# HKU-BAL/Clair3-RNA

Hardware: NVIDIA B200
Metric: candidate sites/sec (tensor+inference) (higher is better)
Workload: dtype int32 pileup + fp16/fp32-accumulate network

## Files before the change

### clair3_rna_b200/csrc/c3r_abi.cu

```cuda
#include <cstdio>
#include <cstdlib>
#include <cstring>
#include <string>
#include <vector>
#include <chrono>
#include <map>
#include <cuda_runtime.h>

#include "../../include/c3r_b200.h"
#include "pileup.cuh"
#include "nn_fp32.cuh"
#include "nn_tc.cuh"
#include "call.cuh"

using namespace c3r;

namespace {

struct Buf {
    void* p = nullptr;
    size_t cap = 0;
};
struct Pin {
    void* p = nullptr;
    size_t cap = 0;
};

constexpr int N_SLOTS = 4;
constexpr int N_EV = 9;

struct Slot {
    bool in_use = false;
    bool has_result = false;
    cudaStream_t st = nullptr;
    cudaStream_t st_a = nullptr;
    cudaEvent_t ev[N_EV] = {};
    cudaEvent_t ev_alt = nullptr;
    cudaEvent_t ev_call[2] = {};
    bool calls = false;
    Buf pos, flag, mapq, hp, cigar_off, cigar, seq_off, seq, ref;
    Buf admit, read_end, op_x, op_y, op_info, blockmax;
    Buf covA, covE, rowR, cov_up, ptile, ctile, csuper, word_base;
    Buf row_pos, counts, row_depth, row_flag, head_cnt, tail_cnt, skipdiff, max_skip, row_ins, row_del;
    Buf binc, bin_cur, events, raw, cov, cov_tile, refnib;
    Buf pbed, cbed, known, covP;
    Buf cand_row, cand_pos, cand_depth, tensor, alt_off, alt_n, alt, cur_ref, deleted, probs;
    Buf d_calls;
    Buf xop;
    bool fused_window = false;
    Buf scalars;
    Buf scan_scratch;
    ScanState scan = {};
    uint32_t scan_epoch = 0;
    size_t zero_bytes = 0;
    bool pending_b = false;
    cudaEvent_t ev_cnt = nullptr;
    uint64_t order = 0;
    int64_t n_seq_bytes = 0, n_known_sites = 0;
    bool exact_bounds = false;
    int deferred_rc = 0;
    std::string deferred_err;
    Pin h_scalars, h_pos, h_depth, h_probs, h_alt_off, h_alt_n, h_alt, h_tensor, h_row_pos, h_counts, h_row_depth, h_calls;
    Dev d;
    int64_t n_rows = 0, n_cand = 0, alt_total = 0;
    int launches = 0;
    c3r_result res;
};

}

struct c3r_ctx {
    int device = 0;
    c3r_params prm;
    std::string err;
    Slot slots[N_SLOTS];
    int sm_count = 148;
    bool have_weights = false;
// ... 57 lines not shown
    CK(cudaMallocHost(&b.p, want));
    b.cap = want;
    return 0;
}
void release(Buf& b) { if (b.p) cudaFree(b.p); b.p = nullptr; b.cap = 0; }
void release(Pin& b) { if (b.p) cudaFreeHost(b.p); b.p = nullptr; b.cap = 0; }

template <class T> T* P(Buf& b) { return (T*)b.p; }

__global__ void __launch_bounds__(128) k_call(const Dev d, const float* __restrict__ probs, int64_t n, c3r_call* __restrict__ out) {
    for (int64_t i = blockIdx.x * (int64_t)blockDim.x + threadIdx.x; i < n; i += (int64_t)gridDim.x * blockDim.x) {
        c3rcall::CallIn c;
        c.e = reinterpret_cast<const c3r_alt_entry*>(d.alt) + d.alt_off[i];
        c.n = d.alt_n[i];
        c.probs = probs + 24 * i;
        c.ref = d.ref;
        c.ref_len = d.ref_len;
        c.p0 = (int64_t)d.cand_pos[i] - (d.ref_start0 + 1);
        c.seq = d.seq;
        c3r_call r;
        c3rcall::decide_call(c, r);
        out[i] = r;
    }
}
static_assert(sizeof(AltEntry) == sizeof(c3r_alt_entry), "AltEntry mirrors c3r_alt_entry");

int run_stage_a(c3r_ctx* ctx, Slot& s) {
    Dev& d = s.d;
    cudaStream_t st = s.st_a;
    int& L = s.launches;
    CK(cudaMemsetAsync(s.covA.p, 0, s.zero_bytes, st));
    CK(cudaMemsetAsync(s.scalars.p, 0, 64, st));
    CK(cudaEventRecord(s.ev[1], st));
    if (d.n_reads > 0) {
        static const int force_g = getenv("C3R_CIGAR_G") ? atoi(getenv("C3R_CIGAR_G")) : 0;
        const int64_t avg = d.n_ops / d.n_reads;
        const int G = force_g ? force_g : avg >= 16 ? 32 : 8;
        if (G == 32) k_cigar<32><<<(unsigned)((d.n_reads * 32 + 255) / 256), 256, 0, st>>>(d);
        else if (G == 16) k_cigar<16><<<(unsigned)((d.n_reads * 16 + 255) / 256), 256, 0, st>>>(d);
        else k_cigar<8><<<(unsigned)((d.n_reads * 8 + 255) / 256), 256, 0, st>>>(d);
        ++L;
    }
    if (d.n_known > 0) { k_mark_known<<<(unsigned)((d.n_known + 255) / 256), 256, 0, st>>>(d); ++L; }
    const unsigned ptiles = (unsigned)((d.NW + PT_WORDS - 1) / PT_WORDS);
    k_row_bits<<<ptiles, 256, 0, st>>>(d); ++L;
    if (d.n_pbed >= 0) { k_bed_mask<<<(unsigned)((d.NW + 4 + 255) / 256), 256, 0, st>>>(d, (uint32_t*)s.covP.p); ++L; }
    if (d.head_tail) {
        k_last_col<<<(unsigned)((d.NW + 255) / 256), 256, 0, st>>>(d);
        k_last_gap<<<(unsigned)((d.NW + 255) / 256), 256, 0, st>>>(d);
        L += 2;
    }
    k_row_rank<<<ptiles, 256, 0, st>>>(d); ++L;
    CK(cudaEventRecord(s.ev[2], st));
    if (d.n_ops > 0) {
        const int64_t chunks = (d.n_ops + CMP_THREADS - 1) / CMP_THREADS;
        const int64_t cap = (int64_t)ctx->sm_count * 6;
        k_cmp<<<(unsigned)(chunks < cap ? chunks : cap), CMP_THREADS, 0, st>>>(d);
        ++L;
    }
    if (d.padding) { OpSkip op; op.d = d; L += device_scan(op, d.L_ub, s.scan, s.scan_epoch, (Int2*)nullptr, st); }
    { OpEvents op; op.d = d; L += device_scan(op, d.L_ub + 1, s.scan, s.scan_epoch, (int32_t*)nullptr, st); }
    if (d.C == 18) k_scatter_aggr<4><<<(unsigned)(ctx->sm_count * 8 + 1), 1024, 0, st>>>(d);
    else k_scatter_aggr<6><<<(unsigned)(ctx->sm_count * 8 + 1), 1024, 0, st>>>(d);
    ++L;
    CK(cudaEventRecord(s.ev[3], st));
    int64_t nb = (d.L_ub + COV_TILE - 1) / COV_TILE;
    {
        const int64_t res = (int64_t)ctx->sm_count * (d.C == 30 ? 4 : 5);
        const unsigned grid = (unsigned)(nb < res ? nb : res);
        if (d.C == 18) k_rows<18><<<grid, ROWS_WARPS * 32, 0, st>>>(d);
        else k_rows<30><<<grid, ROWS_WARPS * 32, 0, st>>>(d);
        ++L;
    }
    CK(cudaEventRecord(s.ev[4], st));
    k_cand_emit<<<(unsigned)(nb < ctx->sm_count * 16 ? nb : ctx->sm_count * 16), 256, 0, st>>>(d); ++L;
    CK(cudaEventRecord(s.ev[5], st));
    CK(cudaGetLastError());
    return 0;
}

int parse_scalars(c3r_ctx* ctx, Slot& s) {
    const int64_t* hs = (const int64_t*)s.h_scalars.p;
    s.n_rows = hs[0];
    s.n_cand = hs[1];
    const int32_t err = ((const int32_t*)s.h_scalars.p)[6];
    if (err == 7)
        return fail(ctx, C3R_ERR_CAPACITY, "a position is covered by more than 8000 reads: samtools mpileup (the reference's "
                                           "column source) caps the depth there and drops reads; this chunk is refused "
                                           "rather than called on different counts");
    if (err) {
// ... 180 lines not shown
        CK(cudaStreamCreateWithPriority(&s.st_a, cudaStreamNonBlocking, prio_lo));
        for (int k = 0; k < N_EV; ++k) CK(cudaEventCreate(&s.ev[k]));
        CK(cudaEventCreateWithFlags(&s.ev_alt, cudaEventDisableTiming));
        for (int k = 0; k < 2; ++k) CK(cudaEventCreate(&s.ev_call[k]));
        CK(cudaEventCreateWithFlags(&s.ev_cnt, cudaEventDisableTiming | (getenv("C3R_BLOCKING_COUNTS") ? cudaEventBlockingSync : 0)));
        if (ensure(ctx, s.scalars, 256)) return C3R_ERR_CUDA;
        if (ensure_pin(ctx, s.h_scalars, 256)) return C3R_ERR_CUDA;
    }
    CK(cudaStreamCreateWithFlags(&ctx->fwd_stream, cudaStreamNonBlocking));
    if (ensure(ctx, ctx->thr, 2 * THR_N * sizeof(uint16_t))) return C3R_ERR_CUDA;
    k_thr_table<<<(THR_N + 255) / 256, 256>>>((uint16_t*)ctx->thr.p, (uint16_t*)ctx->thr.p + THR_N, params->snp_min_af, params->indel_min_af);
    CK(cudaGetLastError());
    CK(cudaDeviceSynchronize());
    return C3R_OK;
}

void c3r_destroy(c3r_ctx* ctx) {
    if (!ctx) return;
    if (getenv("C3R_TIMING") && ctx->tc.pipe)
        fprintf(stderr, "[c3r] %ld network passes, %ld with LSTM1 in pieces beside the previous pass\n", ctx->tc.pipe->n_pass, ctx->tc.pipe->n_overlap);
    if (getenv("C3R_TIMING") && ctx->n_submit)
        fprintf(stderr, "[c3r] %lld submits, host ms each: buffers %.3f, h2d calls %.3f, stage A launches %.3f, earlier "
                        "tickets advanced at submit %.3f, deferred part (wait for the counts + stage B + d2h calls) %.3f, - %.3f\n", (long long)ctx->n_submit,
                1e3 * ctx->t_phase[0] / ctx->n_submit, 1e3 * ctx->t_phase[1] / ctx->n_submit, 1e3 * ctx->t_phase[2] / ctx->n_submit,
                1e3 * ctx->t_phase[3] / ctx->n_submit, 1e3 * ctx->t_phase[4] / ctx->n_submit, 1e3 * ctx->t_phase[5] / ctx->n_submit);
    cudaSetDevice(ctx->device);
    cudaDeviceSynchronize();
    if (ctx->nn_done) cudaEventDestroy(ctx->nn_done);
    for (int i = 0; i < N_SLOTS; ++i) {
        Slot& s = ctx->slots[i];
        Buf* bs[] = {&s.pos, &s.flag, &s.mapq, &s.hp, &s.cigar_off, &s.cigar, &s.seq_off, &s.seq, &s.ref, &s.admit,
                     &s.read_end, &s.op_x, &s.op_y, &s.op_info, &s.blockmax, &s.covA, &s.covE, &s.rowR, &s.cov_up, &s.ptile, &s.ctile, &s.csuper,
                     &s.word_base, &s.row_pos, &s.counts, &s.row_depth, &s.row_flag, &s.head_cnt, &s.tail_cnt,
                     &s.skipdiff, &s.max_skip, &s.row_ins, &s.row_del, &s.binc, &s.bin_cur, &s.events, &s.raw, &s.cov, &s.cov_tile, &s.refnib,
                     &s.cand_row, &s.cand_pos, &s.cand_depth, &s.tensor, &s.alt_off, &s.alt_n, &s.alt, &s.cur_ref,
                     &s.deleted, &s.probs, &s.scalars, &s.scan_scratch, &s.pbed, &s.cbed, &s.known, &s.covP, &s.xop, &s.d_calls};
        for (Buf* b : bs) release(*b);
        Pin* ps[] = {&s.h_scalars, &s.h_pos, &s.h_depth, &s.h_probs, &s.h_alt_off, &s.h_alt_n, &s.h_alt, &s.h_tensor,
                     &s.h_row_pos, &s.h_counts, &s.h_row_depth, &s.h_calls};
        for (Pin* b : ps) release(*b);
        for (int k = 0; k < N_EV; ++k) if (s.ev[k]) cudaEventDestroy(s.ev[k]);
        if (s.ev_alt) cudaEventDestroy(s.ev_alt);
        for (int k = 0; k < 2; ++k) if (s.ev_call[k]) cudaEventDestroy(s.ev_call[k]);
        if (s.ev_cnt) cudaEventDestroy(s.ev_cnt);
        if (s.st) cudaStreamDestroy(s.st);
        if (s.st_a) cudaStreamDestroy(s.st_a);
    }
    release(ctx->wbuf);
    release(ctx->nn_scratch);
    release(ctx->fwd_in);
    release(ctx->ref_res);
    release(ctx->refnib_res);
    release(ctx->thr);
    release(ctx->fwd_out);
    tc_release(ctx->tc);
    if (ctx->fwd_stream) cudaStreamDestroy(ctx->fwd_stream);
    delete ctx;
}

int c3r_host_alloc(void** out, int64_t n_bytes) {
    if (!out || n_bytes <= 0) return C3R_ERR_ARG;
    *out = nullptr;
    return cudaHostAlloc(out, (size_t)n_bytes, cudaHostAllocPortable) == cudaSuccess ? C3R_OK : C3R_ERR_CUDA;
}
void c3r_host_free(void* p) { if (p) cudaFreeHost(p); }

const char* c3r_last_error(c3r_ctx* ctx) { return ctx ? ctx->err.c_str() : "null context"; }
// ... 63 lines not shown
    ctx->filter = nullptr;
    return rc;
}

static int size_rows(c3r_ctx* ctx, Slot& s, const uint32_t* cigar_host) {
    Dev& d = s.d;
    int64_t md_len = 0, n_skip = 0, ev_ub = 0;
    if (cigar_host) {
        for (int64_t k = 0; k < d.n_ops; ++k) {
            const uint32_t c = cigar_host[k], op = c & 15u;
            const int64_t len = c >> 4;
            if (op == 0 || op == 2 || op == 7 || op == 8) md_len += len;
            if (op == 3) ++n_skip;
        }
        ev_ub = d.n_ops + 2 * s.n_seq_bytes;
    } else {
        md_len = 4 * s.n_seq_bytes;
        n_skip = d.n_ops;
        ev_ub = d.n_ops + s.n_seq_bytes / 2;
    }
    int64_t L_ub = md_len + 32 * (n_skip + d.n_reads) + 64;
    L_ub += 33 * s.n_known_sites;
    if (L_ub > d.W) L_ub = d.W;
    if (L_ub < 64) L_ub = 64;
    d.L_ub = L_ub;
    d.events_ub = ev_ub + 8;
    d.cand_cap = L_ub;
#define EN(b, bytes) if (ensure(ctx, s.b, (size_t)(bytes))) return C3R_ERR_CUDA
    EN(row_pos, (L_ub + 2) * 4); EN(counts, ((L_ub + 32) * d.C) * 4); EN(row_depth, (L_ub + 2) * 4); EN(row_flag, L_ub + 2);
    EN(head_cnt, (L_ub + 2) * 4); EN(tail_cnt, (L_ub + 2) * 4); EN(skipdiff, (L_ub + 2) * 8); EN(max_skip, (L_ub + 2) * 4);
    EN(row_ins, (L_ub + 2) * 4); EN(row_del, (L_ub + 2) * 4);
    EN(binc, (L_ub + 4) * 4); EN(bin_cur, (L_ub + 4) * 4);
    EN(events, d.events_ub * sizeof(RowEvent)); EN(raw, d.events_ub * sizeof(RowEvent));
    EN(cov, (L_ub + 4) * NCOV_MAX * 4); EN(cov_tile, (L_ub / COV_TILE + 4) * NCOV_MAX * 4);
    EN(ctile, (L_ub / COV_TILE + 4) * 4); EN(csuper, (L_ub / (64 * COV_TILE) + 4) * 4);
    EN(cand_row, (L_ub + 2) * 4); EN(cand_pos, (L_ub + 2) * 4); EN(cand_depth, (L_ub + 2) * 4);
    EN(cur_ref, (L_ub + 2) * 8); EN(deleted, L_ub + 2);
    {
        int64_t mx = d.n_ops > d.NW ? d.n_ops : d.NW;
        if (L_ub + 4 > mx) mx = L_ub + 4;
        const size_t tiles = (size_t)(mx / SCAN_TILE + 2);
        const size_t need = 256 + tiles * 4 + 2 * tiles * sizeof(ScanElem) + 64;
        if (s.scan_scratch.cap < need) {
            EN(scan_scratch, need);
            CK(cudaMemsetAsync(s.scan_scratch.p, 0, s.scan_scratch.cap, s.st_a));
        }
        uint8_t* sp = (uint8_t*)s.scan_scratch.p;
        const size_t cap_tiles = (s.scan_scratch.cap - 256 - 64) / (4 + 2 * sizeof(ScanElem));
        s.scan.ctrl = (unsigned int*)sp;
        s.scan.status = (uint32_t*)(sp + 256);
        s.scan.aggr = sp + 256 + ((cap_tiles * 4 + 15) / 16) * 16;
        s.scan.incl = (uint8_t*)s.scan.aggr + cap_tiles * sizeof(ScanElem);
        s.scan.err = P<int32_t>(s.scalars) + 6;
    }
#undef EN
    d.row_pos = P<int32_t>(s.row_pos); d.counts = P<int32_t>(s.counts); d.row_depth = P<int32_t>(s.row_depth);
    d.row_flag = P<uint8_t>(s.row_flag); d.head_cnt = P<int32_t>(s.head_cnt); d.tail_cnt = P<int32_t>(s.tail_cnt);
    d.skipdiff = P<Int2>(s.skipdiff); d.max_skip = P<int32_t>(s.max_skip);
    d.row_inscnt = P<int32_t>(s.row_ins); d.row_delcnt = P<int32_t>(s.row_del);
    d.binc = P<int32_t>(s.binc); d.bin_cur = P<int32_t>(s.bin_cur);
    d.events = P<RowEvent>(s.events); d.raw = P<RowEvent>(s.raw); d.cov = P<int32_t>(s.cov); d.cov_tile = P<int32_t>(s.cov_tile);
    d.ctile = P<int32_t>(s.ctile); d.csuper = P<int32_t>(s.csuper);
    d.cand_row = P<int32_t>(s.cand_row); d.cand_pos = P<int32_t>(s.cand_pos); d.cand_depth = P<int32_t>(s.cand_depth);
    d.cur_ref = P<Int2>(s.cur_ref); d.deleted = P<uint8_t>(s.deleted);
    return 0;
}

static int submit_once(c3r_ctx* ctx, const c3r_reads* rd, const uint8_t* ref, int64_t ref_start1, int64_t ref_len,
                       int64_t region_start1, int64_t region_end1, c3r_ticket* ticket) {
    if (!ref) {
        if (!ctx->ref_res_len) return fail(ctx, C3R_ERR_STATE, "ref == NULL but c3r_set_reference was never called");
        ref_start1 = ctx->ref_res_start0 + 1;
        ref_len = ctx->ref_res_len;
    }
    if (!ctx->have_weights) return fail(ctx, C3R_ERR_STATE, "c3r_set_weights must be called before c3r_submit_chunk");
    if (region_end1 < region_start1 || region_start1 < 1) return fail(ctx, C3R_ERR_ARG, "bad region");
    if (region_end1 > 0x7fff0000LL) return fail(ctx, C3R_ERR_CAPACITY, "positions must fit int32");
    if (rd->n_seq_bytes * 2 >= 0xffffffffLL) return fail(ctx, C3R_ERR_CAPACITY, "more than 4G bases in one chunk");
    if (rd->n_reads >= (1LL << 28)) return fail(ctx, C3R_ERR_CAPACITY, "more than 2^28 reads in one chunk");
    CK(cudaSetDevice(ctx->device));
    auto now = [] { return std::chrono::duration<double>(std::chrono::steady_clock::now().time_since_epoch()).count(); };
    double tp = now();
    auto lap = [&](int k) { const double t = now(); ctx->t_phase[k] += t - tp; tp = t; };
    ++ctx->n_submit;
    int si = -1;
    for (int i = 0; i < N_SLOTS; ++i) if (!ctx->slots[i].in_use) { si = i; break; }
    if (si < 0) return fail(ctx, C3R_ERR_STATE, "all tickets in flight; c3r_release one first");
    Slot& s = ctx->slots[si];
    s.launches = 0;
    s.has_result = false;
    s.calls = ctx->calls;
    Dev& d = s.d;
    memset(&d, 0, sizeof d);
    const c3r_params& pr = ctx->prm;
// ... 423 lines not shown
```

### clair3_rna_b200/csrc/pileup.cuh

```cuda
#pragma once
#include <cstdint>
#include <cuda_runtime.h>
#include <cuda_fp16.h>
#include "scan.cuh"

namespace c3r {

constexpr int MPILEUP_MAX_DEPTH = 8000;
constexpr int WIN = 33;
constexpr int FLANK = 16;
constexpr int TILE_ROWS = 32;
constexpr int COV_UP = 5;
constexpr int PT_WORDS = 1024;
constexpr uint32_t OP_SKIP = 0xffffffffu;
constexpr int COV_TILE = 256;

struct RowEvent {
    uint32_t info;
    int32_t len;
    uint32_t yb;
    int32_t row;
};

struct AltEntry {
// ... 15 lines not shown
struct Dev {
    int64_t n_reads, n_ops;
    const int32_t* pos; const uint16_t* flag; const uint8_t* mapq; const uint8_t* hp;
    const int32_t* cigar_off; const uint32_t* cigar; const int64_t* seq_off; const uint8_t* seq;
    const uint8_t* ref; int64_t ref_start0; int64_t ref_len;
    int32_t R0, R1; int64_t W; int64_t NW;
    int32_t C; int32_t min_cov; int32_t min_mq; uint32_t excl; double snp_af, indel_af;
    int32_t padding; int32_t max_depth; double skip_prop;
    int32_t dbg;

    const uint16_t* thr_snp; const uint16_t* thr_indel;
    const int32_t* pbed; int32_t n_pbed;
    const int32_t* cbed; int32_t n_cbed;
    const int32_t* known; int32_t n_known;
    const uint32_t* covP; int32_t head_tail;
    int32_t* tail;
    uint8_t* admit; int32_t* read_end;
    int32_t* op_x; uint32_t* op_y;
    uint32_t* op_info;
    uint32_t* covA; uint32_t* covE; uint32_t* rowR; int32_t* word_base;
    uint32_t* upA[COV_UP]; uint32_t* upE[COV_UP];
    int32_t* ptile;
    int32_t* kctr;
    int64_t L_ub;
    int64_t* n_rows;
    int32_t* row_pos; int32_t* counts; int32_t* row_depth; uint8_t* row_flag;
    int32_t* head_cnt; int32_t* tail_cnt; Int2* skipdiff; int32_t* max_skip;
    int32_t* row_inscnt; int32_t* row_delcnt;
    int32_t* binc; int32_t* bin_cur; RowEvent* events;
    RowEvent* raw; int64_t* n_raw;
    int64_t events_ub;
    int32_t* cov;
    int32_t* cov_tile;
    const uint32_t* refnib; int64_t n_ref_words;
    int32_t* blockmax;
    int32_t* ctile;
    int32_t* csuper;
    int64_t* n_cand; int32_t* cand_row; int64_t cand_cap;
    int32_t* cand_pos; int32_t* cand_depth;
    int32_t* tensor;
    int64_t* alt_off; int32_t* alt_n; AltEntry* alt; int64_t alt_cap;
    Int2* cur_ref; uint8_t* deleted;
    int32_t* err;
};

__device__ __forceinline__ bool op_consumes_ref(uint32_t op) { return op == 0 || op == 2 || op == 3 || op == 7 || op == 8; }
__device__ __forceinline__ bool op_consumes_qry(uint32_t op) { return op == 0 || op == 1 || op == 4 || op == 7 || op == 8; }
__device__ __forceinline__ bool op_is_match(uint32_t op) { return op == 0 || op == 7 || op == 8; }

__device__ __forceinline__ int32_t row_lower_bound(const Dev& d, int32_t p) {
    if (p <= d.R0) return 0;
    int64_t o = (int64_t)p - d.R0;
    if (o >= d.W) o = d.W;
    const int64_t w = o >> 5;
    const uint32_t m = (1u << (o & 31)) - 1u;
    return d.word_base[w] + __popc(d.rowR[w] & m);
}
__device__ __forceinline__ bool bit_at(const uint32_t* bm, int64_t o) { return (bm[o >> 5] >> (o & 31)) & 1u; }

__device__ __forceinline__ uint32_t nib_at(const uint8_t* seq, uint32_t q) {
    const uint32_t b = seq[q >> 1];
    return (q & 1u) ? (b & 15u) : (b >> 4);
}
__device__ __forceinline__ int ref_index(const Dev& d, int32_t p, bool* is_acgt) {
    const int64_t o = (int64_t)p - d.ref_start0;
    uint8_t c = (o >= 0 && o < d.ref_len) ? d.ref[o] : (uint8_t)'N';
// ... 253 lines not shown
    if (own) {
        int32_t idx = b;
#pragma unroll
        for (int j = 0; j < 4; ++j) {
            const int32_t p0 = d.R0 + (int32_t)((w4 + j) << 5);
            if (r[j] == 0xffffffffu) {
                for (int q = 0; q < 32; ++q) if (idx + q < d.L_ub) d.row_pos[idx + q] = p0 + q;
                idx += 32;
            } else {
                for (uint32_t m = r[j]; m; m &= m - 1) { if (idx < d.L_ub) d.row_pos[idx] = p0 + __ffs(m) - 1; ++idx; }
            }
        }
    }
    int64_t z0 = tile_base, z1 = tile_end;
    if (blockIdx.x == gridDim.x - 1) z1 += 2;
    if (z1 > d.L_ub + 2) z1 = d.L_ub + 2;
    for (int64_t i = z0 + t; i < z1; i += 256) {
        d.binc[i] = 0;
        d.bin_cur[i] = 0;
        for (int c = 0; c < NC; ++c) d.cov[i * NC + c] = 0;
        if (d.padding) {
            d.head_cnt[i] = 0; d.tail_cnt[i] = 0;
            Int2 z; z.a = 0; z.b = 0;
            d.skipdiff[i] = z;
            d.deleted[i] = 0;
        }
    }
    if (blockIdx.x == 0)
        for (int64_t i = t; i < d.L_ub / (64 * COV_TILE) + 2; i += 256) d.csuper[i] = 0;
    for (int64_t i = z0 / COV_TILE + t; i <= (z1 > z0 ? (z1 - 1) / COV_TILE : z0 / COV_TILE); i += 256) d.ctile[i] = 0;
    if (z1 > z0) {
        const int64_t ct0 = z0 / COV_TILE, ct1 = (z1 - 1) / COV_TILE + 1;
        for (int64_t i = ct0 * NC + t; i < (ct1 + 1) * NC; i += 256) d.cov_tile[i] = 0;
    }
}

__device__ __forceinline__ uint32_t nibmask(int n) {
    uint32_t m;
    asm("shl.b32 %0, 1, %1;" : "=r"(m) : "r"((uint32_t)(n < 0 ? 0 : 4 * n)));
    return m - 1u;
}

__global__ void k_refnib(const uint8_t* __restrict__ ref, int64_t ref_len, uint32_t* __restrict__ out, int64_t n_words) {
    const int64_t w = (int64_t)blockIdx.x * blockDim.x + threadIdx.x;
    if (w >= n_words) return;
    uint32_t v = 0;
#pragma unroll
    for (int j = 0; j < 8; ++j) {
        const int64_t o = w * 8 + j;
        uint8_t c = o < ref_len ? ref[o] : (uint8_t)'N';
        if (c >= 'a') c -= 32;
        const uint32_t nib = c == 'A' ? 1u : c == 'C' ? 2u : c == 'G' ? 4u : c == 'T' ? 8u : 0u;
        v |= nib << (4 * j);
    }
    out[w] = v;
}

constexpr int NCOV_MAX = 6;
constexpr int CMP_THREADS = 256;
constexpr int CMP_STAGE = 1536;

struct __align__(16) CmpOp {
    int32_t w0, w1;
    int32_t kw;
    uint32_t sh;
    int32_t rbase;
// ... 32 lines not shown
    const int32_t wi = w + c.kw;
    uint32_t f0, f1;
    if ((uint32_t)wi < (uint32_t)(d.n_ref_words - 1)) { f0 = d.refnib[wi]; f1 = d.refnib[wi + 1]; }
    else {
        f0 = (wi >= 0 && wi < d.n_ref_words) ? d.refnib[wi] : 0u;
        f1 = (wi + 1 >= 0 && wi + 1 < d.n_ref_words) ? d.refnib[wi + 1] : 0u;
    }
    uint32_t x = rw ^ __funnelshift_r(f0, f1, c.sh);
    x &= (w == c.w0 ? c.m0 : 0xffffffffu) & (w == c.w1 ? c.m1 : 0xffffffffu);
    if (x) cmp_emit(d, st, c, w, rw, x);
}

__device__ __forceinline__ void cmp_flush(const Dev& d, EventStage& st) {
    __syncthreads();
    const int n = st.n < CMP_STAGE ? st.n : CMP_STAGE;
    if (threadIdx.x == 0 && n > 0) st.base = (int)atomicAdd((unsigned long long*)d.n_raw, (unsigned long long)n);
    __syncthreads();
    if (n > 0) {
        const long long base = st.base;
        if (base + n > d.events_ub) { if (threadIdx.x == 0) atomicExch(d.err, 3); }
        else {
            for (int i = threadIdx.x; i < n; i += CMP_THREADS) {
                const RowEvent e = st.buf[i];
                d.raw[base + i] = e;
                atomicAdd(&d.binc[e.row], 1);
            }
        }
    }
    __syncthreads();
    if (threadIdx.x == 0) st.n = 0;
    __syncthreads();
}

__global__ void __launch_bounds__(CMP_THREADS) k_cmp(Dev d) {
    __shared__ EventStage st;
    __shared__ CmpOp wops[CMP_THREADS / 32][32];
    __shared__ int32_t wpre[CMP_THREADS / 32][32];
    const int lane = threadIdx.x & 31;
    const int NC = d.C == 30 ? 6 : 4;
    if (*d.err == 1) return;
    __shared__ int chunk_s;
    if (threadIdx.x == 0) st.n = 0;
    for (;;) {
    if (threadIdx.x == 0) chunk_s = atomicAdd(&d.kctr[3], 1);
    __syncthreads();
    const int64_t k0 = (int64_t)chunk_s * CMP_THREADS;
    if (k0 >= d.n_ops) break;
    const int64_t k = k0 + threadIdx.x;
    CmpOp cmp;
    cmp.w0 = 0; cmp.w1 = -1; cmp.kw = 0; cmp.sh = 0; cmp.rbase = 0; cmp.info = 0; cmp.m0 = 0; cmp.m1 = 0;
    do {
        if (k >= d.n_ops) break;
        const uint32_t oi = d.op_info[k];
        if (oi == OP_SKIP) break;
        const int32_t r = (int32_t)(oi >> 4);
        const uint32_t c = d.cigar[k];
        const uint32_t op = c & 15u;
        const int32_t len = (int32_t)(c >> 4);
        if (!op_consumes_ref(op) || len == 0) break;
        const int32_t x = d.op_x[k];
        const uint32_t rev = oi & 1u;
        const uint32_t hp = (oi >> 2) & 3u;
        const int32_t a = x < d.R0 ? d.R0 : x;
        const int32_t b = x + len > d.R1 ? d.R1 : x + len;

        if (op == 3) {
            if (d.padding && b > a) {
                const int32_t ra = row_lower_bound(d, a), rb = row_lower_bound(d, b);
                if (rb > ra) {
                    int32_t* f = rev ? &d.skipdiff[0].b : &d.skipdiff[0].a;
                    atomicAdd(&f[2 * (int64_t)ra], 1);
                    atomicAdd(&f[2 * (int64_t)rb], -1);
                }
            }
            break;
        }
        if (b > a) {
            const int32_t ra = row_lower_bound(d, a), rb = ra + (b - a);
            const int ch = (op == 2 ? 2 : 0) + (int)rev;
            atomicAdd(d.cov + (int64_t)ra * NC + ch, 1);
            atomicAdd(d.cov + (int64_t)rb * NC + ch, -1);
            const bool hpc = NC == 6 && op != 2 && hp;
            if (hpc) { atomicAdd(d.cov + (int64_t)ra * NC + 3 + hp, 1); atomicAdd(d.cov + (int64_t)rb * NC + 3 + hp, -1); }
            if (ra / COV_TILE != rb / COV_TILE) {
                atomicAdd(d.cov_tile + (int64_t)(ra / COV_TILE) * NC + ch, 1);
                atomicAdd(d.cov_tile + (int64_t)(rb / COV_TILE) * NC + ch, -1);
                if (hpc) {
                    atomicAdd(d.cov_tile + (int64_t)(ra / COV_TILE) * NC + 3 + hp, 1);
                    atomicAdd(d.cov_tile + (int64_t)(rb / COV_TILE) * NC + 3 + hp, -1);
                }
            }
            if (op != 2) {
                const int64_t qa = (int64_t)d.op_y[k] + (a - x);
                const int64_t qb = qa + (b - a);
                cmp.w0 = (int32_t)(qa >> 3); cmp.w1 = (int32_t)((qb - 1) >> 3);
                cmp.m0 = ~nibmask((int)(qa & 7)); cmp.m1 = nibmask((int)(qb - 8 * (int64_t)cmp.w1));
                const int64_t K = ((int64_t)a - d.ref_start0) - qa;
                cmp.kw = (int32_t)(K >> 3);
                cmp.sh = ((uint32_t)K & 7u) * 4u;
                cmp.rbase = (int32_t)((int64_t)ra - qa);
                cmp.info = oi & ~2u;
            }
        }
        if (d.padding) {
            if (x == d.pos[r] && x >= d.R0 && x < d.R1) {
                bool first = true;
                for (int32_t j = d.cigar_off[r]; j < k; ++j)
                    if (op_consumes_ref(d.cigar[j] & 15u) && (d.cigar[j] >> 4)) first = false;
                if (first) atomicAdd(&d.head_cnt[row_lower_bound(d, x)], 1);
            }
            const int32_t end = d.read_end[r];
            if (x + len == end && end - 1 >= d.R0 && end - 1 < d.R1)
                atomicAdd(&d.tail_cnt[row_lower_bound(d, end - 1)], 1);
        }
        const int32_t last = x + len - 1;
        if (last < d.R0 || last >= d.R1) break;
        if (oi & 2u) break;
        int64_t j = k + 1;
        bool more = true;
        int32_t ins_len = 0, del_len = 0;
        const uint32_t op2 = d.cigar[j] & 15u;
        if (op2 != 1 && !(op2 == 2 && op != 2)) break;
        if (op2 == 1) {
            while (more) {
                const uint32_t cj = d.cigar[j], o = cj & 15u;
                if (o == 1) ins_len += (int32_t)(cj >> 4);
                else if (o != 6) break;
                more = !(d.op_info[j] & 2u);
                ++j;
            }
        }
        if (more && (d.cigar[j] & 15u) == 2 && op != 2) {
            while (more) {
                const uint32_t cj = d.cigar[j];
                if ((cj & 15u) != 2) break;
                del_len += (int32_t)(cj >> 4);
                more = !(d.op_info[j] & 2u);
                ++j;
            }
        }
        if (!ins_len && !del_len) break;
        const int32_t row = row_lower_bound(d, last);
        for (int which = 0; which < 2; ++which) {
            const int32_t l = which ? del_len : ins_len;
            if (!l) continue;
            emit_event(d, st, row, ((uint32_t)r << 4) | (hp << 2) | ((uint32_t)which << 1) | rev, l,
                       d.op_y[k] + (op_is_match(op) ? (uint32_t)len : 0u));
        }
    } while (0);

    {
        const int warp = threadIdx.x >> 5;
        const int32_t cnt = cmp.w1 - cmp.w0 + 1;
        int32_t incl = cnt;
#pragma unroll
        for (int o = 1; o < 32; o <<= 1) { const int32_t y = __shfl_up_sync(0xffffffffu, incl, o); if (lane >= o) incl += y; }
        const int32_t total = __shfl_sync(0xffffffffu, incl, 31);
        wops[warp][lane] = cmp;
        wpre[warp][lane] = incl - cnt;
        __syncwarp();
        for (int32_t g = lane; g < total; g += 32) {
            int i = 0;
#pragma unroll
            for (int stp = 16; stp > 0; stp >>= 1) if (wpre[warp][i + stp] <= g) i += stp;
            const CmpOp c = wops[warp][i];
            cmp_one(d, st, c, c.w0 + (g - wpre[warp][i]));
        }
    }
    __syncthreads();
    const bool fl = st.n >= CMP_STAGE / 2;
    __syncthreads();
    if (fl) cmp_flush(d, st);
    }
    cmp_flush(d, st);
}

struct OpEvents {
    typedef int32_t T;
    struct Ctx {};
    Dev d;
    __device__ void ctx_init(Ctx&) const {}
    __device__ T identity() const { return 0; }
    __device__ T combine(const T& x, const T& y) const { return x + y; }
    __device__ int64_t size() const { return *d.n_rows + 1; }
    __device__ T load(int64_t i) const { return d.binc[i]; }
    __device__ void store(int64_t i, const T& incl, const T& own, Ctx&) const { d.binc[i] = incl - own; }
};
struct OpSkip {
    typedef Int2 T;
    struct Ctx {};
    Dev d;
    __device__ void ctx_init(Ctx&) const {}
    __device__ T identity() const { T t; t.a = 0; t.b = 0; return t; }
    __device__ T combine(const T& x, const T& y) const { T t; t.a = x.a + y.a; t.b = x.b + y.b; return t; }
    __device__ int64_t size() const { return *d.n_rows; }
    __device__ T load(int64_t i) const { return d.skipdiff[i]; }
    __device__ void store(int64_t i, const T& incl, const T&, Ctx&) const {
        int32_t m = incl.a > incl.b ? incl.a : incl.b;
        const int32_t h = d.head_cnt[i], t = d.tail_cnt[i];
        m = m > h ? m : h;
        m = m > t ? m : t;
        d.max_skip[i] = m;
    }
};

// ... 282 lines not shown
    __shared__ __align__(16) int32_t stage[ROWS_WARPS][TILE_ROWS * C];
    __shared__ uint32_t done_s[ROWS_WARPS][IND_WORDS];
    const int warp = threadIdx.x >> 5, lane = threadIdx.x & 31;
    if (*d.err == 1) return;
    const int64_t L = *d.n_rows;
    const int32_t ev_base = d.binc[0];
    for (int64_t tile = blockIdx.x; tile * COV_TILE < L; tile += gridDim.x) {
        const int64_t base = tile * COV_TILE;
        const int64_t row = base + threadIdx.x;
        const bool live = row < L;
        int32_t carry[NC];
#pragma unroll
        for (int c = 0; c < NC; ++c) carry[c] = d.cov_tile[tile * NC + c];
        int32_t cv[NC];
#pragma unroll
        for (int c = 0; c < NC; ++c) cv[c] = 0;
        int32_t p = 0, e0 = 0, e1 = 0;
        uint8_t rc = (uint8_t)'N';
        if (live) {
            if (NC == 4) { const int4 t = *(const int4*)(d.cov + row * 4); cv[0] = t.x; cv[1] = t.y; cv[2] = t.z; cv[3] = t.w; }
            else {
                const int2* q = (const int2*)(d.cov + row * 6);
                const int2 t0 = q[0], t1 = q[1], t2 = q[2];
                cv[0] = t0.x; cv[1] = t0.y; cv[2] = t1.x; cv[3] = t1.y; cv[NC - 2] = t2.x; cv[NC - 1] = t2.y;
            }
            p = d.row_pos[row];
            e0 = d.binc[row] - ev_base; e1 = d.binc[row + 1] - ev_base;
            const int64_t ro = (int64_t)p - d.ref_start0;
            if (ro >= 0 && ro < d.ref_len) rc = d.ref[ro];
        }
        int32_t pre[NC];
#pragma unroll
        for (int c = 0; c < NC; ++c) pre[c] = 0;
        for (int w = 0; w < warp; ++w) {
            const int64_t rw = base + w * 32 + lane;
            if (rw >= L) continue;
            if (NC == 4) { const int4 t = *(const int4*)(d.cov + rw * 4); pre[0] += t.x; pre[1] += t.y; pre[2] += t.z; pre[3] += t.w; }
            else {
                const int2* q = (const int2*)(d.cov + rw * 6);
                const int2 t0 = q[0], t1 = q[1], t2 = q[2];
                pre[0] += t0.x; pre[1] += t0.y; pre[2] += t1.x; pre[3] += t1.y; pre[NC - 2] += t2.x; pre[NC - 1] += t2.y;
            }
        }
#pragma unroll
        for (int c = 0; c < NC; ++c) {
            int32_t x = cv[c];
#pragma unroll
            for (int o = 1; o < 32; o <<= 1) { const int32_t y = __shfl_up_sync(0xffffffffu, x, o); if (lane >= o) x += y; }
            int32_t b = pre[c];
#pragma unroll
            for (int o = 16; o > 0; o >>= 1) b += __shfl_xor_sync(0xffffffffu, b, o);
            cv[c] = x + b + carry[c];
        }
        int32_t* v = &stage[warp][lane * C];
        constexpr int KA = C == 30 ? 20 : 10;
        static_assert(KA <= C, "the counters of a row fit its slice of the staging tile");
#pragma unroll
        for (int i = 0; i < KA; ++i) v[i] = 0;
        const int32_t E1w = __reduce_max_sync(0xffffffffu, live ? e1 : 0);
        const int32_t E0w = min(__reduce_min_sync(0xffffffffu, live ? e0 : 0x7fffffff), E1w);
        const int32_t ev_row0 = (int32_t)(base + warp * 32);
        uint32_t indel_rows = 0;
        __syncwarp();
        for (int32_t s = E0w + lane; s < E1w; s += 32) {
            const RowEvent e = d.events[s];
            const int rl = e.row - ev_row0;
            if (e.len != 0) indel_rows |= 1u << rl;
            else if (e.yb <= 4u) {
                int32_t* a = &stage[warp][rl * C];
                atomicAdd(&a[(e.info & 1u) * 5 + e.yb], 1);
                if (C == 30) {
                    const uint32_t hp = (e.info >> 2) & 3u;
                    if (hp == 1 || hp == 2) atomicAdd(&a[10 + (hp - 1) * 5 + e.yb], 1);
                }
// ... 526 lines not shown
```

Baseline: 10.75 million.

## Process CIGAR ops per read in lane groups and add per-warp coverage deltas

The compare kernel now assigns each read to a group of G lanes that walk its CIGAR ops cooperatively. Ballots and shuffles find run openers, merged coverage spans, first-op heads and indel lengths, so each op no longer rescans the read's earlier ops or calls a row binary search. Adjacent same-class ops are merged into one coverage difference pair. A new per-32-row cov_w delta array lets k_rows take the preceding-warp prefix with one load, replacing a loop over earlier warps. The cost is more atomics into cov_w and more complex group-level code that may diverge on irregular CIGARs.

```diff
diff --git a/clair3_rna_b200/csrc/c3r_abi.cu b/clair3_rna_b200/csrc/c3r_abi.cu
--- a/clair3_rna_b200/csrc/c3r_abi.cu
+++ b/clair3_rna_b200/csrc/c3r_abi.cu
@@ -42,7 +42,7 @@
     Buf admit, read_end, op_x, op_y, op_info, blockmax;
     Buf covA, covE, rowR, cov_up, ptile, ctile, csuper, word_base;
     Buf row_pos, counts, row_depth, row_flag, head_cnt, tail_cnt, skipdiff, max_skip, row_ins, row_del;
-    Buf binc, bin_cur, events, raw, cov, cov_tile, refnib;
+    Buf binc, bin_cur, events, raw, cov, cov_tile, cov_w, refnib;
     Buf pbed, cbed, known, covP;
     Buf cand_row, cand_pos, cand_depth, tensor, alt_off, alt_n, alt, cur_ref, deleted, probs;
     Buf d_calls;
@@ -166,10 +166,9 @@
     CK(cudaMemsetAsync(s.covA.p, 0, s.zero_bytes, st));
     CK(cudaMemsetAsync(s.scalars.p, 0, 64, st));
     CK(cudaEventRecord(s.ev[1], st));
+    static const int force_g = getenv("C3R_CIGAR_G") ? atoi(getenv("C3R_CIGAR_G")) : 0;
+    const int G = force_g ? force_g : d.n_reads > 0 && d.n_ops / d.n_reads >= 16 ? 32 : 8;
     if (d.n_reads > 0) {
-        static const int force_g = getenv("C3R_CIGAR_G") ? atoi(getenv("C3R_CIGAR_G")) : 0;
-        const int64_t avg = d.n_ops / d.n_reads;
-        const int G = force_g ? force_g : avg >= 16 ? 32 : 8;
         if (G == 32) k_cigar<32><<<(unsigned)((d.n_reads * 32 + 255) / 256), 256, 0, st>>>(d);
         else if (G == 16) k_cigar<16><<<(unsigned)((d.n_reads * 16 + 255) / 256), 256, 0, st>>>(d);
         else k_cigar<8><<<(unsigned)((d.n_reads * 8 + 255) / 256), 256, 0, st>>>(d);
@@ -187,9 +186,12 @@
     k_row_rank<<<ptiles, 256, 0, st>>>(d); ++L;
     CK(cudaEventRecord(s.ev[2], st));
     if (d.n_ops > 0) {
-        const int64_t chunks = (d.n_ops + CMP_THREADS - 1) / CMP_THREADS;
+        const int64_t chunks = (d.n_reads * G + CMP_THREADS * CMP_READS - 1) / (CMP_THREADS * CMP_READS);
         const int64_t cap = (int64_t)ctx->sm_count * 6;
-        k_cmp<<<(unsigned)(chunks < cap ? chunks : cap), CMP_THREADS, 0, st>>>(d);
+        const unsigned grid = (unsigned)(chunks < cap ? chunks : cap);
+        if (G == 32) k_cmp<32><<<grid, CMP_THREADS, 0, st>>>(d);
+        else if (G == 16) k_cmp<16><<<grid, CMP_THREADS, 0, st>>>(d);
+        else k_cmp<8><<<grid, CMP_THREADS, 0, st>>>(d);
         ++L;
     }
     if (d.padding) { OpSkip op; op.d = d; L += device_scan(op, d.L_ub, s.scan, s.scan_epoch, (Int2*)nullptr, st); }
@@ -436,7 +438,7 @@
         Buf* bs[] = {&s.pos, &s.flag, &s.mapq, &s.hp, &s.cigar_off, &s.cigar, &s.seq_off, &s.seq, &s.ref, &s.admit,
                      &s.read_end, &s.op_x, &s.op_y, &s.op_info, &s.blockmax, &s.covA, &s.covE, &s.rowR, &s.cov_up, &s.ptile, &s.ctile, &s.csuper,
                      &s.word_base, &s.row_pos, &s.counts, &s.row_depth, &s.row_flag, &s.head_cnt, &s.tail_cnt,
-                     &s.skipdiff, &s.max_skip, &s.row_ins, &s.row_del, &s.binc, &s.bin_cur, &s.events, &s.raw, &s.cov, &s.cov_tile, &s.refnib,
+                     &s.skipdiff, &s.max_skip, &s.row_ins, &s.row_del, &s.binc, &s.bin_cur, &s.events, &s.raw, &s.cov, &s.cov_tile, &s.cov_w, &s.refnib,
                      &s.cand_row, &s.cand_pos, &s.cand_depth, &s.tensor, &s.alt_off, &s.alt_n, &s.alt, &s.cur_ref,
                      &s.deleted, &s.probs, &s.scalars, &s.scan_scratch, &s.pbed, &s.cbed, &s.known, &s.covP, &s.xop, &s.d_calls};
         for (Buf* b : bs) release(*b);
@@ -566,7 +568,7 @@
     EN(row_ins, (L_ub + 2) * 4); EN(row_del, (L_ub + 2) * 4);
     EN(binc, (L_ub + 4) * 4); EN(bin_cur, (L_ub + 4) * 4);
     EN(events, d.events_ub * sizeof(RowEvent)); EN(raw, d.events_ub * sizeof(RowEvent));
-    EN(cov, (L_ub + 4) * NCOV_MAX * 4); EN(cov_tile, (L_ub / COV_TILE + 4) * NCOV_MAX * 4);
+    EN(cov, (L_ub + 4) * NCOV_MAX * 4); EN(cov_tile, (L_ub / COV_TILE + 4) * NCOV_MAX * 4); EN(cov_w, (L_ub / TILE_ROWS + 16) * NCOV_MAX * 4);
     EN(ctile, (L_ub / COV_TILE + 4) * 4); EN(csuper, (L_ub / (64 * COV_TILE) + 4) * 4);
     EN(cand_row, (L_ub + 2) * 4); EN(cand_pos, (L_ub + 2) * 4); EN(cand_depth, (L_ub + 2) * 4);
     EN(cur_ref, (L_ub + 2) * 8); EN(deleted, L_ub + 2);
@@ -593,7 +595,7 @@
     d.skipdiff = P<Int2>(s.skipdiff); d.max_skip = P<int32_t>(s.max_skip);
     d.row_inscnt = P<int32_t>(s.row_ins); d.row_delcnt = P<int32_t>(s.row_del);
     d.binc = P<int32_t>(s.binc); d.bin_cur = P<int32_t>(s.bin_cur);
-    d.events = P<RowEvent>(s.events); d.raw = P<RowEvent>(s.raw); d.cov = P<int32_t>(s.cov); d.cov_tile = P<int32_t>(s.cov_tile);
+    d.events = P<RowEvent>(s.events); d.raw = P<RowEvent>(s.raw); d.cov = P<int32_t>(s.cov); d.cov_tile = P<int32_t>(s.cov_tile); d.cov_w = P<int32_t>(s.cov_w);
     d.ctile = P<int32_t>(s.ctile); d.csuper = P<int32_t>(s.csuper);
     d.cand_row = P<int32_t>(s.cand_row); d.cand_pos = P<int32_t>(s.cand_pos); d.cand_depth = P<int32_t>(s.cand_depth);
     d.cur_ref = P<Int2>(s.cur_ref); d.deleted = P<uint8_t>(s.deleted);
diff --git a/clair3_rna_b200/csrc/pileup.cuh b/clair3_rna_b200/csrc/pileup.cuh
--- a/clair3_rna_b200/csrc/pileup.cuh
+++ b/clair3_rna_b200/csrc/pileup.cuh
@@ -71,6 +71,7 @@
     int64_t events_ub;
     int32_t* cov;
     int32_t* cov_tile;
+    int32_t* cov_w;
     const uint32_t* refnib; int64_t n_ref_words;
     int32_t* blockmax;
     int32_t* ctile;
@@ -390,6 +391,8 @@
     if (z1 > z0) {
         const int64_t ct0 = z0 / COV_TILE, ct1 = (z1 - 1) / COV_TILE + 1;
         for (int64_t i = ct0 * NC + t; i < (ct1 + 1) * NC; i += 256) d.cov_tile[i] = 0;
+        const int64_t cw0 = z0 / TILE_ROWS, cw1 = (z1 - 1) / TILE_ROWS + 1;
+        for (int64_t i = cw0 * NC + t; i < (cw1 + 1) * NC; i += 256) d.cov_w[i] = 0;
     }
 }
 
@@ -488,145 +491,228 @@
     __syncthreads();
 }
 
+__device__ __forceinline__ void cov_pair(const Dev& d, int NC, int cls, int32_t xs, int32_t ra, int32_t xe, uint32_t rev, uint32_t hp) {
+    const int32_t a = xs < d.R0 ? d.R0 : xs;
+    const int32_t b = xe > d.R1 ? d.R1 : xe;
+    if (b <= a) return;
+    const int32_t rb = ra + (b - a);
+    const int ch = (cls == 2 ? 2 : 0) + (int)rev;
+    const bool hpc = NC == 6 && cls == 1 && hp;
+    atomicAdd(d.cov + (int64_t)ra * NC + ch, 1);
+    atomicAdd(d.cov + (int64_t)rb * NC + ch, -1);
+    if (hpc) { atomicAdd(d.cov + (int64_t)ra * NC + 3 + hp, 1); atomicAdd(d.cov + (int64_t)rb * NC + 3 + hp, -1); }
+    if (ra / TILE_ROWS != rb / TILE_ROWS) {
+        atomicAdd(d.cov_w + (int64_t)(ra / TILE_ROWS) * NC + ch, 1);
+        atomicAdd(d.cov_w + (int64_t)(rb / TILE_ROWS) * NC + ch, -1);
+        if (hpc) {
+            atomicAdd(d.cov_w + (int64_t)(ra / TILE_ROWS) * NC + 3 + hp, 1);
+            atomicAdd(d.cov_w + (int64_t)(rb / TILE_ROWS) * NC + 3 + hp, -1);
+        }
+    }
+    if (ra / COV_TILE != rb / COV_TILE) {
+        atomicAdd(d.cov_tile + (int64_t)(ra / COV_TILE) * NC + ch, 1);
+        atomicAdd(d.cov_tile + (int64_t)(rb / COV_TILE) * NC + ch, -1);
+        if (hpc) {
+            atomicAdd(d.cov_tile + (int64_t)(ra / COV_TILE) * NC + 3 + hp, 1);
+            atomicAdd(d.cov_tile + (int64_t)(rb / COV_TILE) * NC + 3 + hp, -1);
+        }
+    }
+}
+
+__device__ __noinline__ void indel_walk(const Dev& d, int64_t k, int64_t b, bool anchor_del, uint32_t* ins_len, uint32_t* del_len) {
+    uint32_t il = 0, dl = 0;
+    int64_t j = k + 1;
+    bool more = true;
+    const uint32_t op2 = d.cigar[j] & 15u;
+    if (op2 == 1) {
+        while (more) {
+            const uint32_t cj = d.cigar[j], o = cj & 15u;
+            if (o == 1) il += cj >> 4;
+            else if (o != 6) break;
+            more = j + 1 < b;
+            ++j;
+        }
+    }
+    if ((op2 == 1 || op2 == 2) && more && (d.cigar[j] & 15u) == 2 && !anchor_del) {
+        while (more) {
+            const uint32_t cj = d.cigar[j];
+            if ((cj & 15u) != 2) break;
+            dl += cj >> 4;
+            more = j + 1 < b;
+            ++j;
+        }
+    }
+    *ins_len = il; *del_len = dl;
+}
+
+template <int G>
+__device__ __forceinline__ void cmp_read(const Dev& d, EventStage& st, CmpOp* gops, int32_t* gpre, int64_t r, int NC) {
+    const int gl = threadIdx.x & (G - 1);
+    const int sh = threadIdx.x & 31 & ~(G - 1);
+    const uint32_t gmask = G == 32 ? 0xffffffffu : (((1u << G) - 1u) << sh);
+    const uint32_t gm = G == 32 ? 0xffffffffu : (1u << G) - 1u;
+    const uint32_t below = (1u << gl) - 1u;
+    const int32_t a = d.cigar_off[r], b = d.cigar_off[r + 1];
+    if (b <= a) return;
+    const uint32_t oi = d.op_info[a];
+    if (oi == OP_SKIP) return;
+    const uint32_t info = oi & ~2u;
+    const uint32_t rev = oi & 1u, hp = (oi >> 2) & 3u;
+    const int32_t read_end = d.padding ? d.read_end[r] : 0;
+    int pc = 0;
+    int32_t rxs = 0, rra = 0, xend = 0;
+    for (int32_t k0 = a; k0 < b; k0 += G) {
+        const int32_t k = k0 + gl;
+        const bool valid = k < b;
+        const uint32_t c = valid ? d.cigar[k] : 0u;
+        const uint32_t op = c & 15u;
+        const int32_t len = (int32_t)(c >> 4);
+        const int32_t x = valid ? d.op_x[k] : 0;
+        const uint32_t y = valid ? d.op_y[k] : 0u;
+        const bool refc = valid && op_consumes_ref(op) && len;
+        const int cls = !refc ? 0 : op_is_match(op) ? 1 : op == 2 ? 2 : 3;
+        const uint32_t mNT = (__ballot_sync(gmask, refc) >> sh) & gm;
+        const uint32_t mM = (__ballot_sync(gmask, cls == 1) >> sh) & gm;
+        const uint32_t mD = (__ballot_sync(gmask, cls == 2) >> sh) & gm;
+        const uint32_t ntb = mNT & below;
+        const int pl = ntb ? 31 - __clz(ntb) : -1;
+        const int pcl = pl < 0 ? pc : ((mM >> pl) & 1u) ? 1 : ((mD >> pl) & 1u) ? 2 : 3;
+        const bool opener = refc && cls != pcl;
+        int32_t ra_open = 0;
+        if (opener && cls != 3) ra_open = row_lower_bound(d, x < d.R0 ? d.R0 : x);
+        const uint32_t mO = (__ballot_sync(gmask, opener) >> sh) & gm;
+        const uint32_t oin = mO & (below | (1u << gl)), oex = mO & below;
+        const int li = oin ? 31 - __clz(oin) : gl, le = oex ? 31 - __clz(oex) : gl;
+        int32_t xs_i = __shfl_sync(gmask, x, li, G), ra_i = __shfl_sync(gmask, ra_open, li, G);
+        int32_t xs_e = __shfl_sync(gmask, x, le, G), ra_e = __shfl_sync(gmask, ra_open, le, G);
+        if (!oin) { xs_i = rxs; ra_i = rra; }
+        if (!oex) { xs_e = rxs; ra_e = rra; }
+        if (opener && (pcl == 1 || pcl == 2)) cov_pair(d, NC, pcl, xs_e, ra_e, x, rev, hp);
+
+        const uint32_t mI = (__ballot_sync(gmask, valid && op == 1) >> sh) & gm;
+        const uint32_t mIP = mI | ((__ballot_sync(gmask, valid && op == 6) >> sh) & gm);
+        const uint32_t mDo = (__ballot_sync(gmask, valid && op == 2) >> sh) & gm;
+        uint32_t pI = op == 1 && valid ? (uint32_t)len : 0u, pD = op == 2 && valid ? (uint32_t)len : 0u;
+#pragma unroll
+        for (int o = 1; o < G; o <<= 1) {
+            const uint32_t ui = __shfl_up_sync(gmask, pI, o, G), ud = __shfl_up_sync(gmask, pD, o, G);
+            if (gl >= o) { pI += ui; pD += ud; }
+        }
+        const uint32_t above = gl >= 31 ? 0u : gm & ~((2u << gl) - 1u);
+        const bool nxt_i = gl + 1 < G && ((mI >> (gl + 1)) & 1u);
+        const bool nxt_d = gl + 1 < G && ((mDo >> (gl + 1)) & 1u);
+        const uint32_t eI = gm & ~mIP & above;
+        const int e = eI ? __ffs(eI) - 1 : G;
+        const int s = nxt_i ? e : gl + 1;
+        const bool dchain = cls == 1 && (nxt_i || nxt_d) && s < G && ((mDo >> s) & 1u);
+        const uint32_t fD = dchain ? gm & ~mDo & ~((2u << s) - 1u) : 0u;
+        const int f = fD ? __ffs(fD) - 1 : G;
+        const uint32_t pI_e = __shfl_sync(gmask, pI, nxt_i ? e - 1 : gl, G);
+        const uint32_t pD_f = __shfl_sync(gmask, pD, dchain ? f - 1 : gl, G);
+        const uint32_t pD_s = __shfl_sync(gmask, pD, dchain ? s - 1 : gl, G);
+
+        const int32_t ra_base = xs_i < d.R0 ? d.R0 : xs_i;
+        const int32_t oa = x < d.R0 ? d.R0 : x;
+        const int32_t ob = x + len > d.R1 ? d.R1 : x + len;
+        CmpOp cmp;
+        cmp.w0 = 0; cmp.w1 = -1; cmp.kw = 0; cmp.sh = 0; cmp.rbase = 0; cmp.info = 0; cmp.m0 = 0; cmp.m1 = 0;
+        if (cls == 3) {
+            if (d.padding && ob > oa) {
+                const int32_t rna = row_lower_bound(d, oa), rnb = row_lower_bound(d, ob);
+                if (rnb > rna) {
+                    int32_t* fp = rev ? &d.skipdiff[0].b : &d.skipdiff[0].a;
+                    atomicAdd(&fp[2 * (int64_t)rna], 1);
+                    atomicAdd(&fp[2 * (int64_t)rnb], -1);
+                }
+            }
+        } else if (cls != 0) {
+            if (cls == 1 && ob > oa) {
+                const int32_t ra = ra_i + (oa - ra_base);
+                const int64_t qa = (int64_t)y + (oa - x);
+                const int64_t qb = qa + (ob - oa);
+                cmp.w0 = (int32_t)(qa >> 3); cmp.w1 = (int32_t)((qb - 1) >> 3);
+                cmp.m0 = ~nibmask((int)(qa & 7)); cmp.m1 = nibmask((int)(qb - 8 * (int64_t)cmp.w1));
+                const int64_t K = ((int64_t)oa - d.ref_start0) - qa;
+                cmp.kw = (int32_t)(K >> 3);
+                cmp.sh = ((uint32_t)K & 7u) * 4u;
+                cmp.rbase = (int32_t)((int64_t)ra - qa);
+                cmp.info = info;
+            }
+            if (d.padding) {
+                if (pcl == 0 && x >= d.R0 && x < d.R1) atomicAdd(&d.head_cnt[row_lower_bound(d, x)], 1);
+                if (x + len == read_end && read_end - 1 >= d.R0 && read_end - 1 < d.R1)
+                    atomicAdd(&d.tail_cnt[row_lower_bound(d, read_end - 1)], 1);
+            }
+            const int32_t last = x + len - 1;
+            if (last >= d.R0 && last < d.R1 && k + 1 < b && (nxt_i || (nxt_d && cls == 1) || gl == G - 1)) {
+                uint32_t il, dl;
+                const bool cross = k0 + G < b && (gl == G - 1 || (nxt_i && e == G) || (dchain && f == G));
+                if (cross) indel_walk(d, k, b, cls == 2, &il, &dl);
+                else {
+                    il = nxt_i ? pI_e - pI : 0u;
+                    dl = dchain ? pD_f - pD_s : 0u;
+                }
+                const int32_t row = ra_i + (last - ra_base);
+                const uint32_t yb = y + (cls == 1 ? (uint32_t)len : 0u);
+                if (il) emit_event(d, st, row, info, (int32_t)il, yb);
+                if (dl) emit_event(d, st, row, info | 2u, (int32_t)dl, yb);
+            }
+        }
+
+        {
+            const int32_t cnt = cmp.w1 - cmp.w0 + 1;
+            int32_t incl = cnt;
+#pragma unroll
+            for (int o = 1; o < G; o <<= 1) { const int32_t u = __shfl_up_sync(gmask, incl, o, G); if (gl >= o) incl += u; }
+            const int32_t total = __shfl_sync(gmask, incl, G - 1, G);
+            gops[gl] = cmp;
+            gpre[gl] = incl - cnt;
+            __syncwarp(gmask);
+            for (int32_t g = gl; g < total; g += G) {
+                int i = 0;
+#pragma unroll
+                for (int stp = G / 2; stp > 0; stp >>= 1) if (gpre[i + stp] <= g) i += stp;
+                const CmpOp cw = gops[i];
+                cmp_one(d, st, cw, cw.w0 + (g - gpre[i]));
+            }
+            __syncwarp(gmask);
+        }
+        if (mNT) {
+            const int ln = 31 - __clz(mNT);
+            pc = ((mM >> ln) & 1u) ? 1 : ((mD >> ln) & 1u) ? 2 : 3;
+            xend = __shfl_sync(gmask, x + len, ln, G);
+        }
+        rxs = __shfl_sync(gmask, xs_i, G - 1, G);
+        rra = __shfl_sync(gmask, ra_i, G - 1, G);
+    }
+    if (gl == 0 && (pc == 1 || pc == 2)) cov_pair(d, NC, pc, rxs, rra, xend, rev, hp);
+}
+
+constexpr int CMP_READS = 2;
+template <int G>
 __global__ void __launch_bounds__(CMP_THREADS) k_cmp(Dev d) {
     __shared__ EventStage st;
     __shared__ CmpOp wops[CMP_THREADS / 32][32];
     __shared__ int32_t wpre[CMP_THREADS / 32][32];
-    const int lane = threadIdx.x & 31;
+    __shared__ int chunk_s;
+    constexpr int GROUPS = CMP_THREADS / G;
+    const int warp = threadIdx.x >> 5, sh = threadIdx.x & 31 & ~(G - 1);
     const int NC = d.C == 30 ? 6 : 4;
     if (*d.err == 1) return;
-    __shared__ int chunk_s;
     if (threadIdx.x == 0) st.n = 0;
     for (;;) {
-    if (threadIdx.x == 0) chunk_s = atomicAdd(&d.kctr[3], 1);
-    __syncthreads();
-    const int64_t k0 = (int64_t)chunk_s * CMP_THREADS;
-    if (k0 >= d.n_ops) break;
-    const int64_t k = k0 + threadIdx.x;
-    CmpOp cmp;
-    cmp.w0 = 0; cmp.w1 = -1; cmp.kw = 0; cmp.sh = 0; cmp.rbase = 0; cmp.info = 0; cmp.m0 = 0; cmp.m1 = 0;
-    do {
-        if (k >= d.n_ops) break;
-        const uint32_t oi = d.op_info[k];
-        if (oi == OP_SKIP) break;
-        const int32_t r = (int32_t)(oi >> 4);
-        const uint32_t c = d.cigar[k];
-        const uint32_t op = c & 15u;
-        const int32_t len = (int32_t)(c >> 4);
-        if (!op_consumes_ref(op) || len == 0) break;
-        const int32_t x = d.op_x[k];
-        const uint32_t rev = oi & 1u;
-        const uint32_t hp = (oi >> 2) & 3u;
-        const int32_t a = x < d.R0 ? d.R0 : x;
-        const int32_t b = x + len > d.R1 ? d.R1 : x + len;
-
-        if (op == 3) {
-            if (d.padding && b > a) {
-                const int32_t ra = row_lower_bound(d, a), rb = row_lower_bound(d, b);
-                if (rb > ra) {
-                    int32_t* f = rev ? &d.skipdiff[0].b : &d.skipdiff[0].a;
-                    atomicAdd(&f[2 * (int64_t)ra], 1);
-                    atomicAdd(&f[2 * (int64_t)rb], -1);
-                }
-            }
-            break;
-        }
-        if (b > a) {
-            const int32_t ra = row_lower_bound(d, a), rb = ra + (b - a);
-            const int ch = (op == 2 ? 2 : 0) + (int)rev;
-            atomicAdd(d.cov + (int64_t)ra * NC + ch, 1);
-            atomicAdd(d.cov + (int64_t)rb * NC + ch, -1);
-            const bool hpc = NC == 6 && op != 2 && hp;
-            if (hpc) { atomicAdd(d.cov + (int64_t)ra * NC + 3 + hp, 1); atomicAdd(d.cov + (int64_t)rb * NC + 3 + hp, -1); }
-            if (ra / COV_TILE != rb / COV_TILE) {
-                atomicAdd(d.cov_tile + (int64_t)(ra / COV_TILE) * NC + ch, 1);
-                atomicAdd(d.cov_tile + (int64_t)(rb / COV_TILE) * NC + ch, -1);
-                if (hpc) {
-                    atomicAdd(d.cov_tile + (int64_t)(ra / COV_TILE) * NC + 3 + hp, 1);
-                    atomicAdd(d.cov_tile + (int64_t)(rb / COV_TILE) * NC + 3 + hp, -1);
-                }
-            }
-            if (op != 2) {
-                const int64_t qa = (int64_t)d.op_y[k] + (a - x);
-                const int64_t qb = qa + (b - a);
-                cmp.w0 = (int32_t)(qa >> 3); cmp.w1 = (int32_t)((qb - 1) >> 3);
-                cmp.m0 = ~nibmask((int)(qa & 7)); cmp.m1 = nibmask((int)(qb - 8 * (int64_t)cmp.w1));
-                const int64_t K = ((int64_t)a - d.ref_start0) - qa;
-                cmp.kw = (int32_t)(K >> 3);
-                cmp.sh = ((uint32_t)K & 7u) * 4u;
-                cmp.rbase = (int32_t)((int64_t)ra - qa);
-                cmp.info = oi & ~2u;
-            }
-        }
-        if (d.padding) {
-            if (x == d.pos[r] && x >= d.R0 && x < d.R1) {
-                bool first = true;
-                for (int32_t j = d.cigar_off[r]; j < k; ++j)
-                    if (op_consumes_ref(d.cigar[j] & 15u) && (d.cigar[j] >> 4)) first = false;
-                if (first) atomicAdd(&d.head_cnt[row_lower_bound(d, x)], 1);
-            }
-            const int32_t end = d.read_end[r];
-            if (x + len == end && end - 1 >= d.R0 && end - 1 < d.R1)
-                atomicAdd(&d.tail_cnt[row_lower_bound(d, end - 1)], 1);
-        }
-        const int32_t last = x + len - 1;
-        if (last < d.R0 || last >= d.R1) break;
-        if (oi & 2u) break;
-        int64_t j = k + 1;
-        bool more = true;
-        int32_t ins_len = 0, del_len = 0;
-        const uint32_t op2 = d.cigar[j] & 15u;
-        if (op2 != 1 && !(op2 == 2 && op != 2)) break;
-        if (op2 == 1) {
-            while (more) {
-                const uint32_t cj = d.cigar[j], o = cj & 15u;
-                if (o == 1) ins_len += (int32_t)(cj >> 4);
-                else if (o != 6) break;
-                more = !(d.op_info[j] & 2u);
-                ++j;
-            }
-        }
-        if (more && (d.cigar[j] & 15u) == 2 && op != 2) {
-            while (more) {
-                const uint32_t cj = d.cigar[j];
-                if ((cj & 15u) != 2) break;
-                del_len += (int32_t)(cj >> 4);
-                more = !(d.op_info[j] & 2u);
-                ++j;
-            }
-        }
-        if (!ins_len && !del_len) break;
-        const int32_t row = row_lower_bound(d, last);
-        for (int which = 0; which < 2; ++which) {
-            const int32_t l = which ? del_len : ins_len;
-            if (!l) continue;
-            emit_event(d, st, row, ((uint32_t)r << 4) | (hp << 2) | ((uint32_t)which << 1) | rev, l,
-                       d.op_y[k] + (op_is_match(op) ? (uint32_t)len : 0u));
-        }
-    } while (0);
-
-    {
-        const int warp = threadIdx.x >> 5;
-        const int32_t cnt = cmp.w1 - cmp.w0 + 1;
-        int32_t incl = cnt;
-#pragma unroll
-        for (int o = 1; o < 32; o <<= 1) { const int32_t y = __shfl_up_sync(0xffffffffu, incl, o); if (lane >= o) incl += y; }
-        const int32_t total = __shfl_sync(0xffffffffu, incl, 31);
-        wops[warp][lane] = cmp;
-        wpre[warp][lane] = incl - cnt;
-        __syncwarp();
-        for (int32_t g = lane; g < total; g += 32) {
-            int i = 0;
-#pragma unroll
-            for (int stp = 16; stp > 0; stp >>= 1) if (wpre[warp][i + stp] <= g) i += stp;
-            const CmpOp c = wops[warp][i];
-            cmp_one(d, st, c, c.w0 + (g - wpre[warp][i]));
-        }
-    }
-    __syncthreads();
-    const bool fl = st.n >= CMP_STAGE / 2;
-    __syncthreads();
-    if (fl) cmp_flush(d, st);
+        if (threadIdx.x == 0) chunk_s = atomicAdd(&d.kctr[3], 1);
+        __syncthreads();
+        const int64_t r0 = (int64_t)chunk_s * (GROUPS * CMP_READS);
+        if (r0 >= d.n_reads) break;
+        for (int i = 0; i < CMP_READS; ++i) {
+            const int64_t r = r0 + (int64_t)(threadIdx.x / G) * CMP_READS + i;
+            if (r < d.n_reads) cmp_read<G>(d, st, &wops[warp][sh], &wpre[warp][sh], r, NC);
+        }
+        __syncthreads();
+        const bool fl = st.n >= CMP_STAGE / 2;
+        __syncthreads();
+        if (fl) cmp_flush(d, st);
     }
     cmp_flush(d, st);
 }
@@ -975,14 +1061,13 @@
         int32_t pre[NC];
 #pragma unroll
         for (int c = 0; c < NC; ++c) pre[c] = 0;
-        for (int w = 0; w < warp; ++w) {
-            const int64_t rw = base + w * 32 + lane;
-            if (rw >= L) continue;
-            if (NC == 4) { const int4 t = *(const int4*)(d.cov + rw * 4); pre[0] += t.x; pre[1] += t.y; pre[2] += t.z; pre[3] += t.w; }
+        if (lane < warp) {
+            const int64_t g = tile * ROWS_WARPS + lane;
+            if (NC == 4) { const int4 t = *(const int4*)(d.cov_w + g * 4); pre[0] = t.x; pre[1] = t.y; pre[2] = t.z; pre[3] = t.w; }
             else {
-                const int2* q = (const int2*)(d.cov + rw * 6);
+                const int2* q = (const int2*)(d.cov_w + g * 6);
                 const int2 t0 = q[0], t1 = q[1], t2 = q[2];
-                pre[0] += t0.x; pre[1] += t0.y; pre[2] += t1.x; pre[3] += t1.y; pre[NC - 2] += t2.x; pre[NC - 1] += t2.y;
+                pre[0] = t0.x; pre[1] = t0.y; pre[2] = t1.x; pre[3] = t1.y; pre[NC - 2] = t2.x; pre[NC - 1] = t2.y;
             }
         }
 #pragma unroll
```

Measured after the change: 10.36 million, median of 6. 0.964x the previous value.
